# Yuming-Yang/FactorModeling

Hardware: AMD Instinct MI355X
Metric: factor·asset·days/s (ops+IC+select) (higher is better)
Workload: dtype f64

## Files before the change

factormodeling_amd/csrc/ts_ops.hip:

```cpp
#include <cstdlib>

#include "fmx_common.hpp"

namespace fmx {

__device__ __forceinline__ bool fin(double v) { return __builtin_fabs(v) < __builtin_inf(); }
__device__ __forceinline__ double prep(double v) { return fin(v) ? v : qnan(); }
__device__ __forceinline__ bool pair_ok(double x, double y) { return fin(x) && fin(y); }

struct SumSt {
  double s, ca, cr, prev;
  int n, same;
  __device__ void init(double first) { s = ca = cr = 0.0; n = 0; same = 0; prev = first; }
  __device__ void add(double v) {
    if (fin(v)) {
      n += 1;
      double y = v - ca, t = s + y;
      ca = t - s - y; s = t;
      if (v == prev) same += 1; else same = 1;
      prev = v;
    }
  }
  __device__ void remove(double v) {
    if (fin(v)) {
      n -= 1;
      double y = -v - cr, t = s + y;
      cr = t - s - y; s = t;
    }
  }
  __device__ double result(int64_t minp) const {
    if (n == 0 && minp == 0) return 0.0;
    if (n >= minp) return (same >= n) ? prev * (double)n : s;
    return qnan();
  }
};

struct MeanSt {
  double s, ca, cr, prev;
  int n, neg, same;
  __device__ void init(double first) { s = ca = cr = 0.0; n = neg = same = 0; prev = first; }
  __device__ void add(double v) { if (fin(v)) add_ok(v); }
  __device__ void remove(double v) { if (fin(v)) remove_ok(v); }
  __device__ void add_ok(double v) {
    n += 1;
    double y = v - ca, t = s + y;
    ca = t - s - y; s = t;
    if (__builtin_signbit(v)) neg += 1;
    if (v == prev) same += 1; else same = 1;
    prev = v;
  }
  __device__ void remove_ok(double v) {
    n -= 1;
    double y = -v - cr, t = s + y;
    cr = t - s - y; s = t;
    if (__builtin_signbit(v)) neg -= 1;
  }
  template <class RT>
  __device__ double result_r(int64_t minp, RT rt) const {
    if (n >= minp && n > 0) {
      double r = mdiv(s, (double)n, rt[n]);
      if (same >= n) r = prev;
      else if (neg == 0 && r < 0) r = 0.0;
      else if (neg == n && r > 0) r = 0.0;
      return r;
    }
    return qnan();
  }
  __device__ double result(int64_t minp) const {
    if (n >= minp && n > 0) {
      double r = s / (double)n;
      if (same >= n) r = prev;
      else if (neg == 0 && r < 0) r = 0.0;
      else if (neg == n && r > 0) r = 0.0;
      return r;
    }
    return qnan();
  }
};

struct VarSt {
  double mean, ssq, n, ca, cr, prev;
  int same;
  __device__ void init(double first) { mean = ssq = n = ca = cr = 0.0; same = 0; prev = first; }
  __device__ void add(double v) { if (fin(v)) add_ok(v); }
  __device__ void remove(double v) { if (fin(v)) remove_ok(v); }
  __device__ void add_ok(double v) {
    n += 1.0;
    if (v == prev) same += 1; else same = 1;
    prev = v;
    double pm = mean - ca;
    double y = v - ca;
    double t = y - mean;
    ca = t + mean - y;
    if (n != 0.0) mean = mean + t / n; else mean = 0.0;
    ssq = ssq + (v - pm) * (v - mean);
  }
  __device__ void remove_ok(double v) {
    n -= 1.0;
    if (n != 0.0) {
      double pm = mean - cr;
      double y = v - cr;
      double t = y - mean;
      cr = t + mean - y;
      mean = mean - t / n;
      ssq = ssq - (v - pm) * (v - mean);
    } else {
      mean = 0.0;
      ssq = 0.0;
    }
  }
  template <class RT>
  __device__ void add_r(double v, RT rt) { if (fin(v)) add_ok_r(v, rt); }
  template <class RT>
  __device__ void remove_r(double v, RT rt) { if (fin(v)) remove_ok_r(v, rt); }
  template <class RT>
  __device__ void add_ok_r(double v, RT rt) {
    n += 1.0;
    if (v == prev) same += 1; else same = 1;
    prev = v;
    double pm = mean - ca;
    double y = v - ca;
    double t = y - mean;
    ca = t + mean - y;
    mean = mean + mdiv(t, n, rt[(int)n]);
    ssq = ssq + (v - pm) * (v - mean);
  }
  template <class RT>
  __device__ void remove_ok_r(double v, RT rt) {
    n -= 1.0;
    if (n != 0.0) {
      double pm = mean - cr;
      double y = v - cr;
      double t = y - mean;
      cr = t + mean - y;
      mean = mean - mdiv(t, n, rt[(int)n]);
      ssq = ssq - (v - pm) * (v - mean);
    } else {
      mean = 0.0;
      ssq = 0.0;
    }
  }
  template <class RT>
  __device__ double var_r(int64_t minp, int ddof, RT rt) const {
    if (minp < 1) minp = 1;
    if (n >= (double)minp && n > (double)ddof) {
      if (n == 1.0 || (double)same >= n) return 0.0;
      return mdiv(ssq, n - (double)ddof, rt[(int)n - ddof]);
    }
    return qnan();
  }
  __device__ double var(int64_t minp, int ddof) const {
    if (minp < 1) minp = 1;
    if (n >= (double)minp && n > (double)ddof) {
      if (n == 1.0 || (double)same >= n) return 0.0;
      return ssq / (n - (double)ddof);
    }
    return qnan();
  }
};

struct MVSt {
  double s, cam, crm;
  double mean, ssq, cav, crv;
  double prev;
  int n, neg, same;
  __device__ void init(double first) {
    s = cam = crm = mean = ssq = cav = crv = 0.0;
    n = neg = same = 0;
    prev = first;
  }
  template <class RT>
  __device__ void add_r(double v, RT rt) { if (fin(v)) add_ok_r(v, rt); }
  template <class RT>
  __device__ void remove_r(double v, RT rt) { if (fin(v)) remove_ok_r(v, rt); }
  template <class RT>
  __device__ void add_ok_r(double v, RT rt) {
    n += 1;
    const double y = v - cam, t = s + y;
    cam = t - s - y; s = t;
    if (__builtin_signbit(v)) neg += 1;
    if (v == prev) same += 1; else same = 1;
    prev = v;
    const double pm = mean - cav;
    const double y2 = v - cav;
    const double t2 = y2 - mean;
    cav = t2 + mean - y2;
    mean = mean + mdiv(t2, (double)n, rt[n]);
    ssq = ssq + (v - pm) * (v - mean);
  }
  template <class RT>
  __device__ void remove_ok_r(double v, RT rt) {
    n -= 1;
    const double y = -v - crm, t = s + y;
    crm = t - s - y; s = t;
    if (__builtin_signbit(v)) neg -= 1;
    if (n != 0) {
      const double pm = mean - crv;
      const double y2 = v - crv;
      const double t2 = y2 - mean;
      crv = t2 + mean - y2;
      mean = mean - mdiv(t2, (double)n, rt[n]);
      ssq = ssq - (v - pm) * (v - mean);
    } else {
      mean = 0.0;
      ssq = 0.0;
    }
  }
  template <class RT>
  __device__ double mean_r(int64_t minp, RT rt) const {
    if (n >= minp && n > 0) {
      double r = mdiv(s, (double)n, rt[n]);
      if (same >= n) r = prev;
      else if (neg == 0 && r < 0) r = 0.0;
      else if (neg == n && r > 0) r = 0.0;
      return r;
    }
    return qnan();
  }
  template <class RT>
  __device__ double var_r(int64_t minp, int ddof, RT rt) const {
    if (minp < 1) minp = 1;
    if (n >= minp && n > ddof) {
      if (n == 1 || same >= n) return 0.0;
      return mdiv(ssq, (double)(n - ddof), rt[n - ddof]);
    }
    return qnan();
  }
};

__device__ __forceinline__ double zsqrt(double v) { return v < 0 ? 0.0 : sqrt(v); }

#ifndef TS_DECAY_SPLIT
#define TS_DECAY_SPLIT 1
#endif
template <int W>
__device__ __forceinline__ double decay_dot(const double* ring, int q) {
  constexpr int S = TS_DECAY_SPLIT < W ? TS_DECAY_SPLIT : W;
  double a[S];
#pragma unroll
  for (int j = 0; j < S; ++j) a[j] = 0.0;
#pragma unroll
  for (int k = 1; k <= W; ++k) a[(k - 1) % S] = __builtin_fma(ring[(q + k) % W], (double)k, a[(k - 1) % S]);
  if constexpr (S == 1) return a[0];
  else if constexpr (S == 2) return a[0] + a[1];
  else if constexpr (S == 3) return (a[0] + a[1]) + a[2];
  else return (a[0] + a[1]) + (a[2] + a[3]);
}




struct ColState {
  SumSt ss;
  MeanSt ms;
  VarSt vs;
  double last;
  int64_t i;
  int nan_in_win;
  bool first;
  __device__ void init() { i = 0; nan_in_win = 0; first = true; last = qnan(); }
};

template <int OP>
__device__ __forceinline__ double ts_moment(ColState& c, double v, double old, int W) {
  if (c.first) { c.ss.init(v); c.ms.init(v); c.vs.init(v); c.first = false; }
  const bool full = c.i >= W;
  double out;
  if (OP == FMX_TS_SUM) {
    if (full) c.ss.remove(old);
    c.ss.add(v);
    out = c.ss.result(W);
  } else if (OP == FMX_TS_MEAN) {
    if (full) c.ms.remove(old);
    c.ms.add(v);
    out = c.ms.result(W);
  } else if (OP == FMX_TS_STD || OP == FMX_TS_VAR) {
    if (full) c.vs.remove(old);
    c.vs.add(v);
    const double var = c.vs.var(W, 1);
    out = (OP == FMX_TS_VAR) ? var : zsqrt(var);
  } else if (OP == FMX_TS_ZSCORE) {
    if (full) { c.ms.remove(old); c.vs.remove(old); }
    c.ms.add(v); c.vs.add(v);
    const double m = c.ms.result(W);
    double sd = zsqrt(c.vs.var(W, 1));
    if (sd == 0.0) sd = qnan();
    out = (v - m) / sd;
  } else if (OP == FMX_TS_DIFF) {
    out = full ? v - old : qnan();
  } else if (OP == FMX_TS_DELAY) {
    out = full ? old : qnan();
  } else {
    if (v == v) c.last = v;
    out = c.last;
  }
  c.i += 1;
  return out;
}

template <int OP, int W>
__device__ __forceinline__ double ts_step_reg(ColState& c, double v, double* ring, int q) {
  if (c.first) { c.ss.init(v); c.ms.init(v); c.vs.init(v); c.first = false; }
  double old = qnan();
  if (OP != FMX_TS_BACKFILL) {
    if (c.i >= W) old = ring[q];
    ring[q] = v;
  }
  double out;
  if (OP == FMX_TS_SUM) {
    if (c.i >= W) c.ss.remove(old);
    c.ss.add(v);
    out = c.ss.result(W);
  } else if (OP == FMX_TS_MEAN) {
    if (c.i >= W) c.ms.remove(old);
    c.ms.add(v);
    out = c.ms.result(W);
  } else if (OP == FMX_TS_STD || OP == FMX_TS_VAR) {
    if (c.i >= W) c.vs.remove(old);
    c.vs.add(v);
    const double var = c.vs.var(W, 1);
    out = (OP == FMX_TS_VAR) ? var : zsqrt(var);
  } else if (OP == FMX_TS_ZSCORE) {
    if (c.i >= W) { c.ms.remove(old); c.vs.remove(old); }
    c.ms.add(v); c.vs.add(v);
    const double m = c.ms.result(W);
    double sd = zsqrt(c.vs.var(W, 1));
    if (sd == 0.0) sd = qnan();
    out = (v - m) / sd;
  } else if (OP == FMX_TS_RANK || OP == FMX_TS_DECAY) {
    if (c.i >= W && !fin(old)) c.nan_in_win -= 1;
    if (!fin(v)) c.nan_in_win += 1;
    if (c.i + 1 < W || c.nan_in_win > 0) {
      out = qnan();
    } else if (OP == FMX_TS_RANK) {
      int less = 0, eq = 0;
#pragma unroll
      for (int k = 0; k < W; ++k) {
        less += (ring[k] < v);
        eq += (ring[k] == v);
      }
      constexpr double RW = 1.0 / (double)W;
      out = mdiv((double)less + (double)(eq + 1) / 2.0, (double)W, RW);
    } else {
      const double acc = decay_dot<W>(ring, q);
      constexpr double DEN = (double)W * (double)(W + 1) / 2.0, RDEN = 1.0 / DEN;
      out = mdiv(acc, DEN, RDEN);
    }
  } else if (OP == FMX_TS_DIFF) {
    out = (c.i >= W) ? v - old : qnan();
  } else if (OP == FMX_TS_DELAY) {
    out = (c.i >= W) ? old : qnan();
  } else {
    if (v == v) c.last = v;
    out = c.last;
  }
  c.i += 1;
  return out;
}

template <int OP, int W, int PF>
__global__ void __launch_bounds__(256, (OP == FMX_TS_SUM || OP == FMX_TS_ZSCORE) ? 4 : 5)
k_ts_reg(const double* __restrict__ X, double* __restrict__ Y, int64_t F, int64_t D, int64_t A, int64_t ld) {
  static_assert(W % PF == 0, "PF must divide W");
  const int64_t col = (int64_t)blockIdx.x * 256 + threadIdx.x;
  if (col >= F * A) return;
  const int64_t f = col / A, a = col - f * A;
  const double* x = X + f * D * ld + a;
  double* y = Y + f * D * ld + a;
  ColState c;
  c.init();
  double ring[W];
#pragma unroll
  for (int q = 0; q < W; ++q) ring[q] = 0.0;
  double pf[PF];
#pragma unroll
  for (int q = 0; q < PF; ++q) pf[q] = q < D ? x[q * ld] : 0.0;
  const double* xp = x + PF * ld;
  double* yp = y;
  int64_t d0 = 0;
  for (; d0 + W + PF <= D; d0 += W) {
#pragma unroll
    for (int q = 0; q < W; ++q) {
      const double v = pf[q % PF];
      pf[q % PF] = *xp;
      xp += ld;
      *yp = ts_step_reg<OP, W>(c, v, ring, q);
      yp += ld;
    }
  }
  for (; d0 < D; d0 += W) {
#pragma unroll
    for (int q = 0; q < W; ++q) {
      const int64_t d = d0 + q;
      if (d < D) {
        const double v = pf[q % PF];
        if (d + PF < D) pf[q % PF] = *xp;
        xp += ld;
        *yp = ts_step_reg<OP, W>(c, v, ring, q);
        yp += ld;
      }
    }
  }
}

#ifndef TS_SET_WAVES
#define TS_SET_WAVES 4
#endif
#ifndef TS_SET_MV
#define TS_SET_MV 1
#endif
struct SetSt {
#if TS_SET_MV
  MVSt mv;
#else
  MeanSt ms;
  VarSt vs;
#endif
  int64_t i;
  int nan_w, nan_r;
  bool first;
};

template <int W, int WR>
__device__ __forceinline__ void ts_set_step(SetSt& c, double v, double* ring, int q, int64_t off,
                                            double* __restrict__ Ym, double* __restrict__ Ys,
                                            double* __restrict__ Yz, double* __restrict__ Yr,
                                            double* __restrict__ Yd, const double* rt) {
  const bool full = c.i >= W;
  const double old = full ? ring[q] : qnan();
  const double oldr = (WR == W) ? old : ((c.i >= WR) ? ring[(q + W - WR) % W] : qnan());
  ring[q] = v;
#if TS_SET_MV
  if (c.first) { c.mv.init(v); c.first = false; }
  if (full) c.mv.remove_r(old, rt);
  c.mv.add_r(v, rt);
  const double m = c.mv.mean_r(W, rt);
  const double sd = zsqrt(c.mv.var_r(W, 1, rt));
#else
  (void)rt;
  if (c.first) { c.ms.init(v); c.vs.init(v); c.first = false; }
  if (full) { c.ms.remove(old); c.vs.remove(old); }
  c.ms.add(v); c.vs.add(v);
  const double m = c.ms.result(W);
  const double sd = zsqrt(c.vs.var(W, 1));
#endif
  if (Ym) __builtin_nontemporal_store(m, Ym + off);
  if (Ys) __builtin_nontemporal_store(sd, Ys + off);
  if (Yz) __builtin_nontemporal_store((v - m) / (sd == 0.0 ? qnan() : sd), Yz + off);
  if (full && !fin(old)) c.nan_w -= 1;
  if (c.i >= WR && !fin(oldr)) c.nan_r -= 1;
  if (!fin(v)) { c.nan_w += 1; c.nan_r += 1; }
  if (Yr) {
    double o = qnan();
    if (c.i + 1 >= WR && c.nan_r == 0) {
      int less = 0, eq = 0;
#pragma unroll
      for (int k = 0; k < WR; ++k) {
        const double w = ring[(q + W - k) % W];
        less += (w < v);
        eq += (w == v);
      }
      constexpr double RWR = 1.0 / (double)WR;
      o = mdiv((double)less + (double)(eq + 1) / 2.0, (double)WR, RWR);
    }
    __builtin_nontemporal_store(o, Yr + off);
  }
  if (Yd) {
    double o = qnan();
    if (c.i + 1 >= W && c.nan_w == 0) {
      const double acc = decay_dot<W>(ring, q);
      constexpr double DEN = (double)W * (double)(W + 1) / 2.0, RDEN = 1.0 / DEN;
      o = mdiv(acc, DEN, RDEN);
    }
    __builtin_nontemporal_store(o, Yd + off);
  }
  c.i += 1;
  __builtin_amdgcn_sched_barrier(0);
}

template <int W, int WR, int PF, int NT = 256>
__global__ void __launch_bounds__(NT, TS_SET_WAVES)
k_ts_set(const double* __restrict__ X, double* __restrict__ Ym, double* __restrict__ Ys, double* __restrict__ Yz,
         double* __restrict__ Yr, double* __restrict__ Yd, int64_t F, int64_t D, int64_t A, int64_t ld) {
  static_assert(W % PF == 0 && WR >= 1 && WR <= W, "windows");
  __shared__ double rt[W + 1];
  for (int k = threadIdx.x; k <= W; k += NT) rt[k] = 1.0 / (double)k;
  __syncthreads();
  const int64_t col = (int64_t)blockIdx.x * NT + threadIdx.x;
  if (col >= F * A) return;
  const int64_t f = col / A, a = col - f * A;
  const int64_t off0 = f * D * ld + a;
  const double* xp = X + off0;
  SetSt c;
  c.i = 0; c.nan_w = 0; c.nan_r = 0; c.first = true;
  double ring[W];
#pragma unroll
  for (int q = 0; q < W; ++q) ring[q] = 0.0;
  double pf[PF];
#pragma unroll
  for (int q = 0; q < PF; ++q) pf[q] = q < D ? __builtin_nontemporal_load(xp + q * ld) : 0.0;
  xp += PF * ld;
  int64_t off = off0;
  int64_t d0 = 0;
  for (; d0 + W + PF <= D; d0 += W) {
#pragma unroll
    for (int q = 0; q < W; ++q) {
      const double v = pf[q % PF];
      pf[q % PF] = __builtin_nontemporal_load(xp);
      xp += ld;
      ts_set_step<W, WR>(c, v, ring, q, off, Ym, Ys, Yz, Yr, Yd, rt);
      off += ld;
      asm volatile("" : "+v"(off));
    }
  }
  for (; d0 < D; d0 += W) {
#pragma unroll
    for (int q = 0; q < W; ++q) {
      const int64_t d = d0 + q;
      if (d < D) {
        const double v = pf[q % PF];
        if (d + PF < D) pf[q % PF] = __builtin_nontemporal_load(xp);
        xp += ld;
        ts_set_step<W, WR>(c, v, ring, q, off, Ym, Ys, Yz, Yr, Yd, rt);
        off += ld;
      asm volatile("" : "+v"(off));
      }
    }
  }
}

template <int OP, int PF>
__global__ void __launch_bounds__(256)
k_ts_rl(const double* __restrict__ X, double* __restrict__ Y, int64_t F, int64_t D, int64_t A, int64_t ld, int W) {
  const int64_t col = (int64_t)blockIdx.x * 256 + threadIdx.x;
  if (col >= F * A) return;
  const int64_t f = col / A, a = col - f * A;
  const double* x = X + f * D * ld + a;
  double* y = Y + f * D * ld + a;
  ColState c;
  c.init();
  for (int64_t d0 = 0; d0 < D; d0 += PF) {
    double v[PF], o[PF];
#pragma unroll
    for (int q = 0; q < PF; ++q) {
      const int64_t d = d0 + q;
      v[q] = d < D ? x[d * ld] : 0.0;
      o[q] = (d < D && d >= W) ? x[(d - W) * ld] : 0.0;
    }
#pragma unroll
    for (int q = 0; q < PF; ++q) {
      const int64_t d = d0 + q;
      if (d >= D) break;
      y[d * ld] = ts_moment<OP>(c, v[q], o[q], W);
    }
  }
}

__device__ __forceinline__ void ts_mom3_step(ColState& c, double v, double old, int W, double* ym, double* ys,
                                             double* yz) {
  if (c.first) { c.ms.init(v); c.vs.init(v); c.first = false; }
  if (c.i >= W) { c.ms.remove(old); c.vs.remove(old); }
  c.ms.add(v); c.vs.add(v);
  const double m = c.ms.result(W);
  const double sd = zsqrt(c.vs.var(W, 1));
  if (ym) __builtin_nontemporal_store(m, ym);
  if (ys) __builtin_nontemporal_store(sd, ys);
  if (yz) __builtin_nontemporal_store((v - m) / (sd == 0.0 ? qnan() : sd), yz);
  c.i += 1;
}

template <int PF>
__global__ void __launch_bounds__(256)
k_ts_mom3(const double* __restrict__ X, double* __restrict__ Ym, double* __restrict__ Ys, double* __restrict__ Yz,
          int64_t F, int64_t D, int64_t A, int64_t ld, int W, const uint8_t* __restrict__ present) {
  const int64_t col = (int64_t)blockIdx.x * 256 + threadIdx.x;
  if (col >= F * A) return;
  const int64_t f = col / A, a = col - f * A;
  const int64_t base = f * D * ld + a;
  const double* x = X + base;
  double* ym = Ym ? Ym + base : nullptr;
  double* ys = Ys ? Ys + base : nullptr;
  double* yz = Yz ? Yz + base : nullptr;
  ColState c;
  c.init();
  if (!present) {
    for (int64_t d0 = 0; d0 < D; d0 += PF) {
      double v[PF], o[PF];
#pragma unroll
      for (int q = 0; q < PF; ++q) {
        const int64_t d = d0 + q;
        v[q] = d < D ? x[d * ld] : 0.0;
        o[q] = (d < D && d >= W) ? x[(d - W) * ld] : 0.0;
      }
#pragma unroll
      for (int q = 0; q < PF; ++q) {
        const int64_t d = d0 + q;
        if (d >= D) break;
        ts_mom3_step(c, v[q], o[q], W, ym ? ym + d * ld : nullptr, ys ? ys + d * ld : nullptr,
                     yz ? yz + d * ld : nullptr);
      }
    }
    return;
  }
  const uint8_t* pres = present + a;
  int64_t tail = -1;
  double oldv = 0.0;
  for (int64_t d = 0; d < D; ++d) {
    const double v = x[d * ld];
    if (pres[d * ld] == 0) {
      if (ym) ym[d * ld] = qnan();
      if (ys) ys[d * ld] = qnan();
      if (yz) yz[d * ld] = qnan();
      continue;
    }
    if (tail < 0) { tail = d; oldv = v; }
    double old = 0.0;
    if (c.i >= W) {
      old = oldv;
      do { ++tail; } while (pres[tail * ld] == 0);
      oldv = x[tail * ld];
    }
    ts_mom3_step(c, v, old, W, ym ? ym + d * ld : nullptr, ys ? ys + d * ld : nullptr, yz ? yz + d * ld : nullptr);
  }
}

template <int OP, int PF>
__global__ void __launch_bounds__(256)
k_ts_ptr(const double* __restrict__ X, double* __restrict__ Y, int64_t F, int64_t D, int64_t A, int64_t ld, int W,
         const uint8_t* __restrict__ present) {
  const int64_t col = (int64_t)blockIdx.x * 256 + threadIdx.x;
  if (col >= F * A) return;
  const int64_t f = col / A, a = col - f * A;
  const double* x = X + f * D * ld + a;
  double* y = Y + f * D * ld + a;
  const uint8_t* pres = present ? present + a : nullptr;
  ColState c;
  c.init();
  int64_t tail = -1;
  double oldv = 0.0;
  for (int64_t d0 = 0; d0 < D; d0 += PF) {
    double v[PF];
    bool p[PF];
#pragma unroll
    for (int q = 0; q < PF; ++q) {
      const int64_t d = d0 + q;
      v[q] = d < D ? x[d * ld] : 0.0;
      p[q] = d < D && (pres == nullptr || pres[d * ld] != 0);
    }
#pragma unroll
    for (int q = 0; q < PF; ++q) {
      const int64_t d = d0 + q;
      if (d >= D) break;
      if (!p[q]) { y[d * ld] = qnan(); continue; }
      if (tail < 0) { tail = d; oldv = v[q]; }
      double old = 0.0;
      if (OP != FMX_TS_BACKFILL && c.i >= W) {
        old = oldv;
        do { ++tail; } while (pres != nullptr && pres[tail * ld] == 0);
        oldv = x[tail * ld];
      }
      y[d * ld] = ts_moment<OP>(c, v[q], old, W);
    }
  }
}

template <int OP>
__global__ void __launch_bounds__(256)
k_ts_lead_ptr(const double* __restrict__ X, double* __restrict__ Y, int64_t F, int64_t D, int64_t A, int64_t ld,
              int K, const uint8_t* __restrict__ present) {
  const int64_t col = (int64_t)blockIdx.x * 256 + threadIdx.x;
  if (col >= F * A) return;
  const int64_t f = col / A, a = col - f * A;
  const double* x = X + f * D * ld + a;
  double* y = Y + f * D * ld + a;
  const uint8_t* pres = present ? present + a : nullptr;
  int64_t i = 0, tail = -1;
  for (int64_t d = 0; d < D; ++d) {
    y[d * ld] = qnan();
    if (pres != nullptr && pres[d * ld] == 0) continue;
    const double v = x[d * ld];
    if (tail < 0) tail = d;
    if (i >= K) {
      const double ov = x[tail * ld];
      y[tail * ld] = (OP == FMX_TS_DIFF) ? ov - v : v;
      do { ++tail; } while (pres != nullptr && pres[tail * ld] == 0);
    }
    ++i;
  }
}

constexpr int TSW_T = 16;
constexpr int TSW_NANBIT = 0x40000000;

__device__ __forceinline__ int wave_min_i(int v) {
#pragma unroll
  for (int o = 32; o >= 1; o >>= 1) v = min(v, __shfl_xor(v, o, 64));
  return v;
}

template <int OP, int T>
__global__ void __launch_bounds__(256)
k_ts_win(const double* __restrict__ X, double* __restrict__ Y, int64_t F, int64_t D, int64_t A, int64_t ld, int W,
         const uint8_t* __restrict__ present, int64_t achunks, int64_t ntiles) {
  static_assert(T <= 30, "tile bit mask");
  const int lane = threadIdx.x & 63;
  const int64_t wid = (int64_t)blockIdx.x * 4 + (threadIdx.x >> 6);
  const int64_t ac = wid % achunks, rest = wid / achunks;
  const int64_t tile = rest % ntiles, f = rest / ntiles;
  if (f >= F) return;
  const int64_t a = ac * 64 + lane;
  const bool ok = a < A;
  const double* x = X + f * D * ld + (ok ? a : A - 1);
  const uint8_t* pres = present ? present + (ok ? a : A - 1) : nullptr;
  const int Di = (int)D;
  const int d0 = (int)tile * T;
  const int d1 = min(Di, d0 + T);
  unsigned pm = 0;
  double v[T];
#pragma unroll
  for (int t = 0; t < T; ++t) {
    const int d = d0 + t;
    const bool in = d < d1;
    v[t] = (OP == FMX_TS_RANK && in) ? x[(int64_t)d * ld] : 0.0;
    if (in && (pres == nullptr || pres[(int64_t)d * ld] != 0)) pm |= 1u << t;
  }
  int pre, s;
  if (pres == nullptr) {
    pre = min(W - 1, d0);
    s = d0 - pre;
  } else {
    pre = 0;
    s = d0;
    for (int db = d0 - 1;; db -= 8) {
      const bool need = ok && pre < W - 1 && db >= 0;
      if (__ballot(need) == 0) break;
      uint8_t pb[8];
#pragma unroll
      for (int k = 0; k < 8; ++k) pb[k] = (db - k >= 0) ? pres[(int64_t)(db - k) * ld] : 0;
#pragma unroll
      for (int k = 0; k < 8; ++k)
        if (need && pre < W - 1 && pb[k]) { ++pre; s = db - k; }
    }
  }
  double qW[T];
  {
    int q = pre;
#pragma unroll
    for (int t = 0; t < T; ++t) { qW[t] = (double)(q - W); q += (pm >> t) & 1u; }
  }
  double acc[T];
  int s2[T];
#pragma unroll
  for (int t = 0; t < T; ++t) { acc[t] = 0.0; s2[t] = 0; }
  const double Wd = (double)W;
  const int smin = wave_min_i(ok ? s : d0);
  double pd = 0.0;
  for (int db = smin; db < d1; db += 8) {
    double u[8];
    bool pu[8];
#pragma unroll
    for (int k = 0; k < 8; ++k) {
      const int d = db + k;
      u[k] = d < d1 ? x[(int64_t)d * ld] : 0.0;
      pu[k] = d < d1 && d >= s && (pres == nullptr || pres[(int64_t)d * ld] != 0);
    }
#pragma unroll
    for (int k = 0; k < 8; ++k) {
      if (!pu[k]) continue;
      const double uk = prep(u[k]);
#pragma unroll
      for (int t = 0; t < T; ++t) {
        const double kk = pd - qW[t];
        const bool inw = kk >= 1.0 && kk <= Wd;
        if (OP == FMX_TS_DECAY) {
          acc[t] = inw ? __builtin_fma(uk, kk, acc[t]) : acc[t];
        } else {
          const int inc = uk < v[t] ? 2 : (uk == v[t] ? 1 : 0);
          const int nx = (uk != uk) ? (s2[t] | TSW_NANBIT) : (s2[t] + inc);
          s2[t] = inw ? nx : s2[t];
        }
      }
      pd += 1.0;
    }
  }
  if (!ok) return;
  double* y = Y + f * D * ld + a;
  const double den = (double)W * (double)(W + 1) / 2.0;
  const double rden = 1.0 / den, rw = 1.0 / Wd;
#pragma unroll
  for (int t = 0; t < T; ++t) {
    const int d = d0 + t;
    if (d >= d1) break;
    double o = qnan();
    if (((pm >> t) & 1u) && qW[t] >= -1.0) {
      if (OP == FMX_TS_DECAY) o = mdiv(acc[t], den, rden);
      else if (s2[t] < TSW_NANBIT) o = mdiv((double)(s2[t] + 1) / 2.0, Wd, rw);
    }
    y[(int64_t)d * ld] = o;
  }
}

template <int PF, bool FAST>
__global__ void __launch_bounds__(256)
k_ts_cvf_rl(const double* __restrict__ X, const double* __restrict__ C, double* __restrict__ Y, int64_t F,
            int64_t D, int64_t A, int64_t ld, int W) {
  extern __shared__ double rt[];
  if (FAST) {
    for (int k = threadIdx.x; k <= W; k += 256) rt[k] = 1.0 / (double)k;
    __syncthreads();
  }
  const int64_t col = (int64_t)blockIdx.x * 256 + threadIdx.x;
  if (col >= F * A) return;
  const int64_t f = col / A, a = col - f * A;
  const double* x = X + f * D * ld + a;
  const double* cc = C + f * D * ld + a;
  double* y = Y + f * D * ld + a;
  ColState c;
  c.init();
  for (int64_t d0 = 0; d0 < D; d0 += PF) {
    double v[PF], o[PF], cv[PF];
#pragma unroll
    for (int q = 0; q < PF; ++q) {
      const int64_t d = d0 + q;
      v[q] = d < D ? x[d * ld] : 0.0;
      o[q] = (d < D && d >= W) ? x[(d - W) * ld] : 0.0;
      cv[q] = d < D ? __builtin_nontemporal_load(cc + d * ld) : 0.0;
    }
#pragma unroll
// ... 134 lines not shown
  __device__ double operator[](int) const { return r; }
};
#endif
template <bool WC>
__global__ void __launch_bounds__(256)
k_ts_corr_feat(const double* __restrict__ X, const double* __restrict__ Ycol, double* __restrict__ C,
               double* __restrict__ Out, int64_t F, int64_t D, int64_t A, int64_t ld, int64_t y_fstride, int W,
               int64_t nab) {
  extern __shared__ double rt_lds[];
  for (int k = threadIdx.x; k <= W; k += 256) rt_lds[k] = 1.0 / (double)k;
  __syncthreads();
#ifdef CF_DIAG_RT
  const CfDiagRt rt{1.0 / (double)W};
#else
  const double* rt = rt_lds;
#endif
  const int64_t ab = blockIdx.x % nab, fg = blockIdx.x / nab;
  const int64_t f = fg * 4 + (threadIdx.x >> 6), a = ab * 64 + (threadIdx.x & 63);
  if (f >= F || a >= A) return;
  const double* x = X + f * D * ld + a;
  const double* yc = Ycol + f * y_fstride + a;
  double* o = Out + f * D * ld + a;
  double* cp = WC ? C + f * D * ld + a : nullptr;
  MeanSt mxy;
  MVSt sx, sy;
  VarSt vs;
  int64_t i = 0, cnt = 0;
  bool first = true;
  double nx, ny, nxo, nyo;
  auto fetch = [&](int64_t d) {
    const bool in = d < D, old = in && d >= W;
    nx = in ? x[d * ld] : 0.0;
    ny = in ? yc[d * ld] : 0.0;
#ifdef CF_DIAG_NOOLD
    nxo = nx;
    nyo = ny;
    (void)old;
#else
    nxo = old ? x[(d - W) * ld] : 0.0;
    nyo = old ? yc[(d - W) * ld] : 0.0;
#endif
  };
  fetch(0);
  for (int64_t d = 0; d < D; ++d) {
    const double xr = nx, yr = ny, xo = nxo, yo = nyo;
    fetch(d + 1);
    const double xv = xr + 0.0 * yr;
    const double yv = yr + 0.0 * xr;
    const double pv = xv * yv;
    if (first) { mxy.init(pv); sx.init(xv); sy.init(yv); vs.init(xr); first = false; }
    if (i >= W) {
      if (pair_ok(xo, yo)) {
        const double ox = xo + 0.0 * yo, oy = yo + 0.0 * xo;
        mxy.remove_ok(ox * oy); sx.remove_ok_r(ox, rt); sy.remove_ok_r(oy, rt);
        cnt -= 1;
      }
      vs.remove_r(xo, rt);
    }
    if (pair_ok(xr, yr)) {
      mxy.add_ok(pv); sx.add_ok_r(xv, rt); sy.add_ok_r(yv, rt);
      cnt += 1;
    }
    vs.add_r(xr, rt);
    const double cc = (double)cnt;
    const double ratio = cnt >= 2 ? mdiv(cc, cc - 1.0, rt[cnt - 1]) : cc / (cc - 1.0);
    const double num = (mxy.result_r(W, rt) - sx.mean_r(W, rt) * sy.mean_r(W, rt)) * ratio;
    const double pv2 = sx.var_r(W, 1, rt) * sy.var_r(W, 1, rt);
    double sg;
    if constexpr (WC) {
      const double cq = num / sqrt(pv2);
      __builtin_nontemporal_store(cq, cp + d * ld);
      sg = cq > 0.0 ? 1.0 : (cq < 0.0 ? -1.0 : (cq == 0.0 ? 0.0 : cq));
    } else {
      const double cq = num / sqrt(pv2);
      sg = cq > 0.0 ? 1.0 : (cq < 0.0 ? -1.0 : (cq == 0.0 ? 0.0 : cq));
    }
    double sd = zsqrt(vs.var_r(W, 1, rt));
    if (sd == 0.0) sd = qnan();
    __builtin_nontemporal_store(sg * (xr / sd), o + d * ld);
    i += 1;
  }
}

__global__ void k_ts_window0(const double* __restrict__ X, double* __restrict__ Y, int64_t n_total,
                             int op, const uint8_t* __restrict__ present, int64_t DA, int64_t ld) {
  (void)ld;
  int64_t i = (int64_t)blockIdx.x * blockDim.x + threadIdx.x;
  int64_t stride = (int64_t)gridDim.x * blockDim.x;
  for (; i < n_total; i += stride) {
    double v = X[i];
    bool p = present ? present[i % DA] : true;
    double o = (op == FMX_TS_DIFF) ? v - v : v;
    Y[i] = p ? o : qnan();
  }
}

__global__ void __launch_bounds__(256)
k_ts_corr_ptr(const double* __restrict__ X, const double* __restrict__ Ycol, double* __restrict__ Out, int64_t F,
              int64_t D, int64_t A, int64_t ld, int64_t y_fstride, int W, const uint8_t* __restrict__ present) {
  const int64_t col = (int64_t)blockIdx.x * 256 + threadIdx.x;
  if (col >= F * A) return;
  const int64_t f = col / A, a = col - f * A;
  const double* x = X + f * D * ld + a;
  const double* yc = Ycol + f * y_fstride + a;
  double* o = Out + f * D * ld + a;
  const uint8_t* pres = present ? present + a : nullptr;
  MeanSt mxy, mx, my;
  VarSt vx, vy;
  int64_t i = 0, cnt = 0, tail = -1;
  bool first = true;
  for (int64_t d = 0; d < D; ++d) {
    if (pres != nullptr && pres[d * ld] == 0) { o[d * ld] = qnan(); continue; }
    const double xr = x[d * ld], yr = yc[d * ld];
    const double xv = xr + 0.0 * yr;
    const double yv = yr + 0.0 * xr;
    const double pv = xv * yv;
    if (first) { mxy.init(pv); mx.init(xv); my.init(yv); vx.init(xv); vy.init(yv); first = false; tail = d; }
    if (i >= W) {
      const double txr = x[tail * ld], tyr = yc[tail * ld];
      if (pair_ok(txr, tyr)) {
        const double ox = txr + 0.0 * tyr, oy = tyr + 0.0 * txr;
        mxy.remove_ok(ox * oy); mx.remove_ok(ox); my.remove_ok(oy); vx.remove_ok(ox); vy.remove_ok(oy);
        cnt -= 1;
      }
      do { ++tail; } while (pres != nullptr && pres[tail * ld] == 0);
    }
    if (pair_ok(xr, yr)) {
      mxy.add_ok(pv); mx.add_ok(xv); my.add_ok(yv); vx.add_ok(xv); vy.add_ok(yv);
      cnt += 1;
    }
    const double c = (double)cnt;
    const double num = (mxy.result(W) - mx.result(W) * my.result(W)) * (c / (c - 1.0));
    const double den = sqrt(vx.var(W, 1) * vy.var(W, 1));
    o[d * ld] = num / den;
    i += 1;
  }
}

__global__ void __launch_bounds__(256)
k_ts_regression_ptr(const double* __restrict__ Yv, const double* __restrict__ Xv, const uint8_t* __restrict__ valid,
                    double* __restrict__ Out, int64_t D, int64_t A, int64_t ld, int W, int rettype) {
  const int64_t a = (int64_t)blockIdx.x * 256 + threadIdx.x;
  if (a >= A) return;
  MeanSt mx, my, mxx, mxy, myy;
  int64_t i = 0, tail = -1;
  bool first = true;
  for (int64_t d = 0; d < D; ++d) {
    const int64_t off = d * ld + a;
    if (!valid[off]) { Out[off] = qnan(); continue; }
    const double xv = Xv[off], yv = Yv[off];
    if (first) { mx.init(xv); my.init(yv); mxx.init(xv * xv); mxy.init(xv * yv); myy.init(yv * yv); first = false; tail = d; }
    if (i >= W) {
      const double ox = Xv[tail * ld + a], oy = Yv[tail * ld + a];
      mx.remove(ox); my.remove(oy); mxx.remove(ox * ox); mxy.remove(ox * oy); myy.remove(oy * oy);
      do { ++tail; } while (valid[tail * ld + a] == 0);
    }
    mx.add(xv); my.add(yv); mxx.add(xv * xv); mxy.add(xv * yv); myy.add(yv * yv);
    const double Mx = mx.result(W), My = my.result(W);
    const double cov = mxy.result(W) - Mx * My;
    const double var_x = mxx.result(W) - Mx * Mx;
    const double beta = cov / var_x;
    const double alpha = My - beta * Mx;
    const double fitted = alpha + beta * xv;
    double r;
    switch (rettype) {
      case 0: r = yv - fitted; break;
      case 1: r = alpha; break;
      case 2: r = beta; break;
      case 3: r = fitted; break;
      default: {
        const double var_y = myy.result(W) - My * My;
        r = (cov * cov) / (var_x * var_y);
      }
    }
    Out[off] = r;
    i += 1;
  }
}

template <int W, int PF>
static const void* ts_reg_for(int op) {
  switch (op) {
    case FMX_TS_SUM: return (const void*)k_ts_reg<FMX_TS_SUM, W, PF>;
    case FMX_TS_MEAN: return (const void*)k_ts_reg<FMX_TS_MEAN, W, PF>;
    case FMX_TS_STD: return (const void*)k_ts_reg<FMX_TS_STD, W, PF>;
    case FMX_TS_VAR: return (const void*)k_ts_reg<FMX_TS_VAR, W, PF>;
    case FMX_TS_ZSCORE: return (const void*)k_ts_reg<FMX_TS_ZSCORE, W, PF>;
    case FMX_TS_RANK: return (const void*)k_ts_reg<FMX_TS_RANK, W, PF>;
    case FMX_TS_DECAY: return (const void*)k_ts_reg<FMX_TS_DECAY, W, PF>;
    case FMX_TS_DIFF: return (const void*)k_ts_reg<FMX_TS_DIFF, W, PF>;
    case FMX_TS_DELAY: return (const void*)k_ts_reg<FMX_TS_DELAY, W, PF>;
    default: return nullptr;
  }
}

static const void* ts_reg_kernel(int op, int W) {
  switch (W) {
    case 5: return ts_reg_for<5, 5>(op);
    case 10: return ts_reg_for<10, 10>(op);
    case 20: return ts_reg_for<20, 5>(op);
    default: return nullptr;
  }
}

template <int PF>
static const void* ts_col_for(int op, bool ptr) {
  switch (op) {
    case FMX_TS_SUM: return ptr ? (const void*)k_ts_ptr<FMX_TS_SUM, PF> : (const void*)k_ts_rl<FMX_TS_SUM, PF>;
    case FMX_TS_MEAN: return ptr ? (const void*)k_ts_ptr<FMX_TS_MEAN, PF> : (const void*)k_ts_rl<FMX_TS_MEAN, PF>;
    case FMX_TS_STD: return ptr ? (const void*)k_ts_ptr<FMX_TS_STD, PF> : (const void*)k_ts_rl<FMX_TS_STD, PF>;
    case FMX_TS_VAR: return ptr ? (const void*)k_ts_ptr<FMX_TS_VAR, PF> : (const void*)k_ts_rl<FMX_TS_VAR, PF>;
    case FMX_TS_ZSCORE:
      return ptr ? (const void*)k_ts_ptr<FMX_TS_ZSCORE, PF> : (const void*)k_ts_rl<FMX_TS_ZSCORE, PF>;
    case FMX_TS_DIFF: return ptr ? (const void*)k_ts_ptr<FMX_TS_DIFF, PF> : (const void*)k_ts_rl<FMX_TS_DIFF, PF>;
    case FMX_TS_DELAY: return ptr ? (const void*)k_ts_ptr<FMX_TS_DELAY, PF> : (const void*)k_ts_rl<FMX_TS_DELAY, PF>;
    case FMX_TS_BACKFILL: return (const void*)k_ts_ptr<FMX_TS_BACKFILL, PF>;
    default: return nullptr;
  }
}

static fmx_status launch_ts_win(int op, const double* X, double* Y, int64_t F, int64_t D, int64_t A, int64_t ld,
                                int W, const uint8_t* present, hipStream_t st) {
  FMX_ARG(D < (int64_t)1 << 30, "too many dates for the windowed kernel");
  int64_t achunks = ceil_div(A, 64), ntiles = ceil_div(D, TSW_T);
  const int64_t waves = F * ntiles * achunks;
  FMX_ARG(ceil_div(waves, 4) < (int64_t)1 << 31, "panel too large for one windowed launch");
  const void* k = op == FMX_TS_RANK ? (const void*)k_ts_win<FMX_TS_RANK, TSW_T>
                                    : (const void*)k_ts_win<FMX_TS_DECAY, TSW_T>;
  void* args[] = {(void*)&X, (void*)&Y, (void*)&F, (void*)&D, (void*)&A, (void*)&ld, (void*)&W,
                  (void*)&present, (void*)&achunks, (void*)&ntiles};
  FMX_HIP(hipLaunchKernel(k, dim3((unsigned)ceil_div(waves, 4)), dim3(256), args, 0, st));
  return FMX_OK;
}

}

using namespace fmx;

extern "C" fmx_status fmx_ts_op(int32_t op, const double* X, double* Y, int64_t F, int64_t D, int64_t A,
                                int64_t ld, int32_t window, const uint8_t* present, void* stream) {
  FMX_ARG(X && Y, "null panel");
  FMX_ARG(F >= 0 && D >= 0 && A >= 0 && ld >= A, "bad dims");
  FMX_ARG(op >= FMX_TS_SUM && op <= FMX_TS_BACKFILL, "unknown ts op");
  if (F == 0 || D == 0 || A == 0) return FMX_OK;
  hipStream_t st = as_stream(stream);
  int W = window;
  if (op == FMX_TS_BACKFILL) W = 1;
  if (op == FMX_TS_DECAY && W < 1) {
    FMX_HIP(hipMemcpyAsync(Y, X, sizeof(double) * F * D * ld, hipMemcpyDeviceToDevice, st));
    if (present) {
      int64_t n = F * D * ld;
      k_ts_window0<<<(int)std::min<int64_t>(ceil_div(n, 256), 8192), 256, 0, st>>>(X, Y, n, FMX_TS_DELAY, present, D * ld, ld);
      FMX_LAUNCH_CHECK("k_ts_window0");
    }
    return FMX_OK;
  }
  if ((op == FMX_TS_DIFF || op == FMX_TS_DELAY) && W == 0) {
    int64_t n = F * D * ld;
    k_ts_window0<<<(int)std::min<int64_t>(ceil_div(n, 256), 8192), 256, 0, st>>>(X, Y, n, op, present, D * ld, ld);
    FMX_LAUNCH_CHECK("k_ts_window0");
    return FMX_OK;
  }
  const dim3 cgrid((unsigned)ceil_div(F * A, 256));
  if ((op == FMX_TS_DIFF || op == FMX_TS_DELAY) && W < 0) {
    FMX_ARG(W > INT32_MIN, "window out of range");
    int K = -W;
    const void* k = op == FMX_TS_DIFF ? (const void*)k_ts_lead_ptr<FMX_TS_DIFF> : (const void*)k_ts_lead_ptr<FMX_TS_DELAY>;
    void* largs[] = {(void*)&X, (void*)&Y, (void*)&F, (void*)&D, (void*)&A, (void*)&ld, (void*)&K, (void*)&present};
    FMX_HIP(hipLaunchKernel(k, cgrid, dim3(256), largs, 0, st));
    return FMX_OK;
  }
  FMX_ARG(W >= 1, "window must be >= 1");
  if (!present && op != FMX_TS_BACKFILL) {
    const void* kr = ts_reg_kernel(op, W);
    if (kr) {
      void* rargs[] = {(void*)&X, (void*)&Y, (void*)&F, (void*)&D, (void*)&A, (void*)&ld};
      FMX_HIP(hipLaunchKernel(kr, cgrid, dim3(256), rargs, 0, st));
      return FMX_OK;
    }
  }
  if (op == FMX_TS_RANK || op == FMX_TS_DECAY) return launch_ts_win(op, X, Y, F, D, A, ld, W, present, st);
  if (!present && op != FMX_TS_BACKFILL) {
    void* rargs[] = {(void*)&X, (void*)&Y, (void*)&F, (void*)&D, (void*)&A, (void*)&ld, (void*)&W};
    FMX_HIP(hipLaunchKernel(ts_col_for<8>(op, false), cgrid, dim3(256), rargs, 0, st));
    return FMX_OK;
  }
  void* pargs[] = {(void*)&X, (void*)&Y, (void*)&F, (void*)&D, (void*)&A, (void*)&ld, (void*)&W, (void*)&present};
  FMX_HIP(hipLaunchKernel(ts_col_for<8>(op, true), cgrid, dim3(256), pargs, 0, st));
  return FMX_OK;
}

extern "C" fmx_status fmx_ts_set(const double* X, double* Ymean, double* Ystd, double* Yzscore, double* Yrank,
                                 double* Ydecay, int64_t F, int64_t D, int64_t A, int64_t ld, int32_t window,
                                 int32_t rank_window, const uint8_t* present, void* stream) {
  FMX_ARG(X, "null panel");
  FMX_ARG(F >= 0 && D >= 0 && A >= 0 && ld >= A, "bad dims");
  FMX_ARG(window >= 1 && rank_window >= 1, "windows must be >= 1");
  double* outs[5] = {Ymean, Ystd, Yzscore, Yrank, Ydecay};
  for (int k = 0; k < 5; ++k) FMX_ARG(outs[k] != X, "outputs must not alias X");
  if (F == 0 || D == 0 || A == 0) return FMX_OK;
  if (!present && window == 20 && rank_window == 10) {
    void* args[] = {(void*)&X, (void*)&Ymean, (void*)&Ystd, (void*)&Yzscore, (void*)&Yrank, (void*)&Ydecay,
                    (void*)&F, (void*)&D, (void*)&A, (void*)&ld};
    FMX_HIP(hipLaunchKernel((const void*)k_ts_set<20, 10, 5>, dim3((unsigned)ceil_div(F * A, 256)), dim3(256), args, 0,
                            as_stream(stream)));
    return FMX_OK;
  }
  const int32_t ops[5] = {FMX_TS_MEAN, FMX_TS_STD, FMX_TS_ZSCORE, FMX_TS_RANK, FMX_TS_DECAY};
  int k0 = 0;
  if (Ymean || Ystd || Yzscore) {
    int W = window;
    void* args[] = {(void*)&X, (void*)&Ymean, (void*)&Ystd, (void*)&Yzscore, (void*)&F, (void*)&D, (void*)&A,
                    (void*)&ld, (void*)&W, (void*)&present};
    FMX_HIP(hipLaunchKernel((const void*)k_ts_mom3<4>, dim3((unsigned)ceil_div(F * A, 256)), dim3(256), args, 0,
                            as_stream(stream)));
    k0 = 3;
  }
  for (int k = k0; k < 5; ++k) {
    if (!outs[k]) continue;
    fmx_status e = fmx_ts_op(ops[k], X, outs[k], F, D, A, ld, k == 3 ? rank_window : window, present, stream);
    if (e) return e;
  }
  return FMX_OK;
}

extern "C" fmx_status fmx_ts_corr(const double* X, const double* Ycol, double* Out, int64_t F, int64_t D,
                                  int64_t A, int64_t ld, int64_t y_fstride, int32_t window,
                                  const uint8_t* present, void* stream) {
  FMX_ARG(X && Ycol && Out, "null panel");
  FMX_ARG(F >= 0 && D >= 0 && A >= 0 && ld >= A, "bad dims");
  FMX_ARG(window >= 1, "window must be >= 1");
  if (F == 0 || D == 0 || A == 0) return FMX_OK;
  int W = window;
  const dim3 grid((unsigned)ceil_div(F * A, 256));
  if (!present) {
    void* rargs[] = {(void*)&X, (void*)&Ycol, (void*)&Out, (void*)&F, (void*)&D, (void*)&A, (void*)&ld,
                     (void*)&y_fstride, (void*)&W};
    if (W <= TSC_MAXW) {
      int64_t nab = ceil_div(A, 64);
      void* fargs[] = {(void*)&X, (void*)&Ycol, (void*)&Out, (void*)&F, (void*)&D, (void*)&A, (void*)&ld,
                       (void*)&y_fstride, (void*)&W, (void*)&nab};
      FMX_HIP(hipLaunchKernel((const void*)k_ts_corr_fast<2>, dim3((unsigned)(nab * ceil_div(F, 4))), dim3(256),
                              fargs, sizeof(double) * (W + 1), as_stream(stream)));
      return FMX_OK;
    }
    const void* kc = (const void*)k_ts_corr_rl<2>;
    FMX_HIP(hipLaunchKernel(kc, grid, dim3(256), rargs, 0, as_stream(stream)));
    return FMX_OK;
  }
  void* args[] = {(void*)&X, (void*)&Ycol, (void*)&Out, (void*)&F, (void*)&D, (void*)&A, (void*)&ld,
                  (void*)&y_fstride, (void*)&W, (void*)&present};
  FMX_HIP(hipLaunchKernel((const void*)k_ts_corr_ptr, grid, dim3(256), args, 0, as_stream(stream)));
  return FMX_OK;
}

extern "C" fmx_status fmx_ts_corr_vol_feature(const double* X, const double* C, double* Y, int64_t F, int64_t D,
                                              int64_t A, int64_t ld, int32_t window, void* stream) {
  FMX_ARG(X && C && Y, "null panel");
  FMX_ARG(Y != X && Y != C, "output must not alias the inputs");
  FMX_ARG(F >= 0 && D >= 0 && A >= 0 && ld >= A, "bad dims");
  FMX_ARG(window >= 1, "window must be >= 1");
  if (F == 0 || D == 0 || A == 0) return FMX_OK;
  int W = window;
  void* args[] = {(void*)&X, (void*)&C, (void*)&Y, (void*)&F, (void*)&D, (void*)&A, (void*)&ld, (void*)&W};
  const bool fast = W <= TSC_MAXW;
  FMX_HIP(hipLaunchKernel(fast ? (const void*)k_ts_cvf_rl<8, true> : (const void*)k_ts_cvf_rl<8, false>,
                          dim3((unsigned)ceil_div(F * A, 256)), dim3(256), args, fast ? sizeof(double) * (W + 1) : 0,
                          as_stream(stream)));
  return FMX_OK;
}

extern "C" fmx_status fmx_ts_corr_feature(const double* X, const double* Ycol, double* C, double* Y, int64_t F,
                                          int64_t D, int64_t A, int64_t ld, int64_t y_fstride, int32_t window,
                                          void* stream) {
  FMX_ARG(X && Ycol && Y, "null panel");
  FMX_ARG(Y != X && Y != Ycol && (!C || (C != X && C != Ycol && C != Y)), "outputs must not alias the inputs");
  FMX_ARG(F >= 0 && D >= 0 && A >= 0 && ld >= A, "bad dims");
  FMX_ARG(window >= 1 && window <= TSC_MAXW, "window must be in [1, 4096]");
  if (F == 0 || D == 0 || A == 0) return FMX_OK;
  int W = window;
  int64_t nab = ceil_div(A, 64);
  void* args[] = {(void*)&X, (void*)&Ycol, (void*)&C, (void*)&Y, (void*)&F, (void*)&D, (void*)&A, (void*)&ld,
                  (void*)&y_fstride, (void*)&W, (void*)&nab};
  const void* k = C ? (const void*)k_ts_corr_feat<true> : (const void*)k_ts_corr_feat<false>;
  FMX_HIP(hipLaunchKernel(k, dim3((unsigned)(nab * ceil_div(F, 4))), dim3(256), args, sizeof(double) * (W + 1),
                          as_stream(stream)));
  return FMX_OK;
}

extern "C" fmx_status fmx_ts_regression(const double* Yv, const double* Xv, const uint8_t* valid, double* Out,
                                        int64_t D, int64_t A, int64_t ld, int32_t window, int32_t rettype,
                                        void* stream) {
  FMX_ARG(Yv && Xv && valid && Out, "null panel");
  FMX_ARG(D >= 0 && A >= 0 && ld >= A, "bad dims");
  FMX_ARG(window >= 1, "window must be >= 1");
  FMX_ARG(rettype == 0 || rettype == 1 || rettype == 2 || rettype == 3 || rettype == 6, "rettype not implemented");
  if (D == 0 || A == 0) return FMX_OK;
  int W = window;
  int rt = rettype;
  void* args[] = {(void*)&Yv, (void*)&Xv, (void*)&valid, (void*)&Out, (void*)&D, (void*)&A, (void*)&ld,
                  (void*)&W, (void*)&rt};
  FMX_HIP(hipLaunchKernel((const void*)k_ts_regression_ptr, dim3((unsigned)ceil_div(A, 256)), dim3(256), args, 0,
                          as_stream(stream)));
  return FMX_OK;
}
```

Measured before the change: 45.94 billion.

## Pair-load rows as 16-byte vectors with lane swaps and scalar-base addressing in ts_set

In the fused rolling-set kernel, each lane now loads two consecutive days for a pair of adjacent columns as a single 16-byte vector. permlane32_swap then redistributes the values so every lane still processes one column sequentially, and the outputs are swapped back and written as 16-byte nontemporal stores. Addresses are split into a wave-uniform scalar base plus a 32-bit per-lane offset to cut 64-bit VGPR address arithmetic. The host picks the paired variant only when alignment and evenness conditions hold. This adds cross-lane swap instructions and a second code path, and the uint32 offset relies on a host-side range check.

After: 46.10 billion, median of 6. Within noise of the previous version (+0.3%).

```diff
diff --git a/factormodeling_amd/csrc/ts_ops.hip b/factormodeling_amd/csrc/ts_ops.hip
--- a/factormodeling_amd/csrc/ts_ops.hip
+++ b/factormodeling_amd/csrc/ts_ops.hip
@@ -1,4 +1,5 @@
 #include <cstdlib>
+#include <type_traits>
 
 #include "fmx_common.hpp"
 
@@ -421,11 +422,70 @@
   bool first;
 };
 
-template <int W, int WR>
-__device__ __forceinline__ void ts_set_step(SetSt& c, double v, double* ring, int q, int64_t off,
-                                            double* __restrict__ Ym, double* __restrict__ Ys,
-                                            double* __restrict__ Yz, double* __restrict__ Yr,
-                                            double* __restrict__ Yd, const double* rt) {
+#ifndef TS_SET_PAIR
+#define TS_SET_PAIR 1
+#endif
+#ifndef TS_SET_SBASE
+#define TS_SET_SBASE 1
+#endif
+
+struct SetOuts { double* y[5]; };
+enum { TSS_MEAN = 0, TSS_STD, TSS_ZSCORE, TSS_RANK, TSS_DECAY };
+
+#define TS_GLOBAL __attribute__((address_space(1)))
+template <class T, class OffT>
+__device__ __forceinline__ TS_GLOBAL T* ts_at(T* base, int64_t ub, OffT& lo) {
+  using C = std::conditional_t<std::is_const_v<T>, const char, char>;
+  C* row = reinterpret_cast<C*>(base) + ub;
+  if constexpr (sizeof(OffT) == 4) asm volatile("" : "+s"(row), "+v"(lo));
+  return (TS_GLOBAL T*)((TS_GLOBAL C*)row + lo);
+}
+
+typedef double ts_dbl2 __attribute__((ext_vector_type(2)));
+__device__ __forceinline__ void ts_hswap(double& a, double& b) {
+  typedef unsigned u32x2 __attribute__((ext_vector_type(2)));
+  u32x2 ua = __builtin_bit_cast(u32x2, a), ub = __builtin_bit_cast(u32x2, b);
+  const auto lo = __builtin_amdgcn_permlane32_swap(ua.x, ub.x, false, false);
+  const auto hi = __builtin_amdgcn_permlane32_swap(ua.y, ub.y, false, false);
+  ua.x = lo[0]; ub.x = lo[1];
+  ua.y = hi[0]; ub.y = hi[1];
+  a = __builtin_bit_cast(double, ua);
+  b = __builtin_bit_cast(double, ub);
+}
+
+template <class OffT>
+struct SetPut8 {
+  const SetOuts& o;
+  int64_t ub;
+  OffT& lo;
+  __device__ __forceinline__ bool want(int k) const { return o.y[k] != nullptr; }
+  __device__ __forceinline__ void put(int k, double val) const {
+    __builtin_nontemporal_store(val, ts_at(o.y[k], ub, lo));
+  }
+};
+struct SetHold {
+  const SetOuts& o;
+  double* h;
+  __device__ __forceinline__ bool want(int k) const { return o.y[k] != nullptr; }
+  __device__ __forceinline__ void put(int k, double val) const { h[k] = val; }
+};
+template <class OffT>
+struct SetPut16 {
+  const SetOuts& o;
+  int64_t ub;
+  OffT& lo;
+  const double* h;
+  __device__ __forceinline__ bool want(int k) const { return o.y[k] != nullptr; }
+  __device__ __forceinline__ void put(int k, double val) const {
+    double a = h[k], b = val;
+    ts_hswap(a, b);
+    __builtin_nontemporal_store(ts_dbl2{a, b}, (TS_GLOBAL ts_dbl2*)ts_at(o.y[k], ub, lo));
+  }
+};
+
+template <int W, int WR, class Sink>
+__device__ __forceinline__ void ts_set_step(SetSt& c, double v, double* ring, int q, const Sink& out,
+                                            const double* rt) {
   const bool full = c.i >= W;
   const double old = full ? ring[q] : qnan();
   const double oldr = (WR == W) ? old : ((c.i >= WR) ? ring[(q + W - WR) % W] : qnan());
@@ -444,13 +504,13 @@
   const double m = c.ms.result(W);
   const double sd = zsqrt(c.vs.var(W, 1));
 #endif
-  if (Ym) __builtin_nontemporal_store(m, Ym + off);
-  if (Ys) __builtin_nontemporal_store(sd, Ys + off);
-  if (Yz) __builtin_nontemporal_store((v - m) / (sd == 0.0 ? qnan() : sd), Yz + off);
+  if (out.want(TSS_MEAN)) out.put(TSS_MEAN, m);
+  if (out.want(TSS_STD)) out.put(TSS_STD, sd);
+  if (out.want(TSS_ZSCORE)) out.put(TSS_ZSCORE, (v - m) / (sd == 0.0 ? qnan() : sd));
   if (full && !fin(old)) c.nan_w -= 1;
   if (c.i >= WR && !fin(oldr)) c.nan_r -= 1;
   if (!fin(v)) { c.nan_w += 1; c.nan_r += 1; }
-  if (Yr) {
+  if (out.want(TSS_RANK)) {
     double o = qnan();
     if (c.i + 1 >= WR && c.nan_r == 0) {
       int less = 0, eq = 0;
@@ -463,54 +523,90 @@
       constexpr double RWR = 1.0 / (double)WR;
       o = mdiv((double)less + (double)(eq + 1) / 2.0, (double)WR, RWR);
     }
-    __builtin_nontemporal_store(o, Yr + off);
-  }
-  if (Yd) {
+    out.put(TSS_RANK, o);
+  }
+  if (out.want(TSS_DECAY)) {
     double o = qnan();
     if (c.i + 1 >= W && c.nan_w == 0) {
       const double acc = decay_dot<W>(ring, q);
       constexpr double DEN = (double)W * (double)(W + 1) / 2.0, RDEN = 1.0 / DEN;
       o = mdiv(acc, DEN, RDEN);
     }
-    __builtin_nontemporal_store(o, Yd + off);
+    out.put(TSS_DECAY, o);
   }
   c.i += 1;
   __builtin_amdgcn_sched_barrier(0);
 }
 
-template <int W, int WR, int PF, int NT = 256>
+template <int W, int WR, int PF, int NT = 256, bool PAIR = false, class OffT = uint32_t>
 __global__ void __launch_bounds__(NT, TS_SET_WAVES)
 k_ts_set(const double* __restrict__ X, double* __restrict__ Ym, double* __restrict__ Ys, double* __restrict__ Yz,
          double* __restrict__ Yr, double* __restrict__ Yd, int64_t F, int64_t D, int64_t A, int64_t ld) {
-  static_assert(W % PF == 0 && WR >= 1 && WR <= W, "windows");
+  constexpr int TP = PAIR ? 2 * PF : PF;
+  static_assert(W % TP == 0 && WR >= 1 && WR <= W, "windows");
   __shared__ double rt[W + 1];
   for (int k = threadIdx.x; k <= W; k += NT) rt[k] = 1.0 / (double)k;
   __syncthreads();
-  const int64_t col = (int64_t)blockIdx.x * NT + threadIdx.x;
+  const int lane = threadIdx.x & 63, h = PAIR ? lane >> 5 : 0;
+  const int64_t cb = (int64_t)blockIdx.x * NT + 64 * __builtin_amdgcn_readfirstlane((int)(threadIdx.x >> 6));
+  if (cb >= F * A) return;
+  const int64_t f0 = cb / A;
+  const int64_t ub0 = (f0 * D * ld + (cb - f0 * A)) * 8;
+  const int64_t col = PAIR ? cb + 2 * (lane & 31) + h : cb + lane;
   if (col >= F * A) return;
   const int64_t f = col / A, a = col - f * A;
-  const int64_t off0 = f * D * ld + a;
-  const double* xp = X + off0;
+  const int64_t ldb = ld * 8;
+  OffT lo1 = (OffT)((f * D * ld + a) * 8 - ub0);
+  OffT lo2 = (OffT)(lo1 + (OffT)(h * (ldb - 8)));
+  const SetOuts outs{{Ym, Ys, Yz, Yr, Yd}};
   SetSt c;
   c.i = 0; c.nan_w = 0; c.nan_r = 0; c.first = true;
   double ring[W];
 #pragma unroll
   for (int q = 0; q < W; ++q) ring[q] = 0.0;
-  double pf[PF];
-#pragma unroll
-  for (int q = 0; q < PF; ++q) pf[q] = q < D ? __builtin_nontemporal_load(xp + q * ld) : 0.0;
-  xp += PF * ld;
-  int64_t off = off0;
+  double pf[TP];
+  int64_t ub = ub0;
   int64_t d0 = 0;
-  for (; d0 + W + PF <= D; d0 += W) {
-#pragma unroll
-    for (int q = 0; q < W; ++q) {
-      const double v = pf[q % PF];
-      pf[q % PF] = __builtin_nontemporal_load(xp);
-      xp += ld;
-      ts_set_step<W, WR>(c, v, ring, q, off, Ym, Ys, Yz, Yr, Yd, rt);
-      off += ld;
-      asm volatile("" : "+v"(off));
+  if (PAIR && W + TP <= D) {
+    ts_dbl2 p2[PF];
+#pragma unroll
+    for (int q = 0; q < PF; ++q)
+      p2[q] = __builtin_nontemporal_load((TS_GLOBAL const ts_dbl2*)ts_at(X, ub0 + 2 * q * ldb, lo2));
+    for (; d0 + W + TP <= D; d0 += W) {
+#pragma unroll
+      for (int q = 0; q < W; q += 2) {
+        const ts_dbl2 r = p2[(q / 2) % PF];
+        p2[(q / 2) % PF] = __builtin_nontemporal_load((TS_GLOBAL const ts_dbl2*)ts_at(X, ub + TP * ldb, lo2));
+        double v0 = r.x, v1 = r.y;
+        ts_hswap(v0, v1);
+        double hold[5];
+        ts_set_step<W, WR>(c, v0, ring, q, SetHold{outs, hold}, rt);
+        ts_set_step<W, WR>(c, v1, ring, q + 1, SetPut16<OffT>{outs, ub, lo2, hold}, rt);
+        ub += 2 * ldb;
+        asm volatile("" : "+s"(ub));
+      }
+    }
+#pragma unroll
+    for (int q = 0; q < PF; ++q) {
+      double v0 = p2[q].x, v1 = p2[q].y;
+      ts_hswap(v0, v1);
+      pf[2 * q] = v0;
+      pf[2 * q + 1] = v1;
+    }
+  } else {
+#pragma unroll
+    for (int q = 0; q < TP; ++q) pf[q] = q < D ? __builtin_nontemporal_load(ts_at(X, ub0 + q * ldb, lo1)) : 0.0;
+  }
+  if (!PAIR) {
+    for (; d0 + W + TP <= D; d0 += W) {
+#pragma unroll
+      for (int q = 0; q < W; ++q) {
+        const double v = pf[q % TP];
+        pf[q % TP] = __builtin_nontemporal_load(ts_at(X, ub + TP * ldb, lo1));
+        ts_set_step<W, WR>(c, v, ring, q, SetPut8<OffT>{outs, ub, lo1}, rt);
+        ub += ldb;
+        asm volatile("" : "+s"(ub));
+      }
     }
   }
   for (; d0 < D; d0 += W) {
@@ -518,12 +614,11 @@
     for (int q = 0; q < W; ++q) {
       const int64_t d = d0 + q;
       if (d < D) {
-        const double v = pf[q % PF];
-        if (d + PF < D) pf[q % PF] = __builtin_nontemporal_load(xp);
-        xp += ld;
-        ts_set_step<W, WR>(c, v, ring, q, off, Ym, Ys, Yz, Yr, Yd, rt);
-        off += ld;
-      asm volatile("" : "+v"(off));
+        const double v = pf[q % TP];
+        if (d + TP < D) pf[q % TP] = __builtin_nontemporal_load(ts_at(X, ub + TP * ldb, lo1));
+        ts_set_step<W, WR>(c, v, ring, q, SetPut8<OffT>{outs, ub, lo1}, rt);
+        ub += ldb;
+        asm volatile("" : "+s"(ub));
       }
     }
   }
@@ -1264,8 +1359,13 @@
   if (!present && window == 20 && rank_window == 10) {
     void* args[] = {(void*)&X, (void*)&Ymean, (void*)&Ystd, (void*)&Yzscore, (void*)&Yrank, (void*)&Ydecay,
                     (void*)&F, (void*)&D, (void*)&A, (void*)&ld};
-    FMX_HIP(hipLaunchKernel((const void*)k_ts_set<20, 10, 5>, dim3((unsigned)ceil_div(F * A, 256)), dim3(256), args, 0,
-                            as_stream(stream)));
+    bool pair = TS_SET_PAIR != 0 && A % 2 == 0 && ld % 2 == 0 && (uintptr_t)X % 16 == 0;
+    for (int k = 0; k < 5; ++k) pair = pair && (uintptr_t)outs[k] % 16 == 0;
+    const bool o32 = TS_SET_SBASE != 0 && (double)(63 / A + 1) * (double)D * (double)ld * 8.0 + (double)ld * 8.0 + 512.0 < 4294967296.0;
+    const void* k = !pair ? (const void*)k_ts_set<20, 10, 5, 256, false, int64_t>
+                          : (o32 ? (const void*)k_ts_set<20, 10, 5, 256, true, uint32_t>
+                                 : (const void*)k_ts_set<20, 10, 2, 256, true, int64_t>);
+    FMX_HIP(hipLaunchKernel(k, dim3((unsigned)ceil_div(F * A, 256)), dim3(256), args, 0, as_stream(stream)));
     return FMX_OK;
   }
   const int32_t ops[5] = {FMX_TS_MEAN, FMX_TS_STD, FMX_TS_ZSCORE, FMX_TS_RANK, FMX_TS_DECAY};
```
